# AY-Liu/Image-Editing-Framework

Hardware: AMD Instinct MI355X
Metric: denoising steps/sec (SD1.5 512x512 P2P edit step, UNet batch 4) (higher is better)
Workload: dtype f16x3; 1 GPU; sd15 UNet (859.5M params) P2P AttentionRefine edit step, 2 prompts x CFG = batch 4, 64x64 latents (512x512 px), 50-step DDIM, guidance 7.5, cross 0.8 / self 0.4, per-step null-text unconditional embeddings (P2P_NTI, edit_real.py); one independent edit per GPU; precision mode f16x3: fp32 storage; every contraction on split operands: hi + lo fp16 halves of each fp32 element, Ah Bh + Al Bh + Ah Bl =

## Files before the change

### image-editing-framework_amd/csrc/cross_p2p_x3.hip

```cpp
#include "ief_common.h"
#include "ief_params.h"
#include "x3_common.h"

template <int D, bool QS = false>
__global__ __launch_bounds__(256, (D > 80) ? 1 : 2) void attn_cross_p2p_x3_kernel(const IefAttnF32Params p, const int* __restrict__ edit_src,
                                                                                  const int* __restrict__ edit_slot,
                                                                                  const float* __restrict__ MT,
                                                                                  const float* __restrict__ coef) {
    constexpr int DG = (D + 15) / 16;
    constexpr int DT = (D + 31) / 32;
    constexpr int KLD = DG * 16 + 8;
    constexpr int VLD = 100;
    constexpr int MLD = 100;
    constexpr float SQ = 1.f, SK = 1.f, SV = 1.f, SP = 16384.f, SM = 256.f;
    const float SPE = p.p_scale > 0.f ? p.p_scale : SP;
    constexpr int RK = 2 * 96 * KLD, RV = 2 * DT * 32 * VLD, RM = 2 * 96 * MLD;
    constexpr int RSZ = RK > RV ? (RK > RM ? RK : RM) : (RV > RM ? RV : RM);
    __shared__ __attribute__((aligned(16))) half_t smem_c[RSZ];
    __shared__ float cf[2 * 96];
    half_t* Kh = smem_c;
    half_t* Kl = Kh + 96 * KLD;
    half_t* Vh = smem_c;
    half_t* Vl = Vh + DT * 32 * VLD;
    half_t* Mh = smem_c;
    half_t* Ml = Mh + 96 * MLD;
    const int tid = threadIdx.x, lane = tid & 63, wid = tid >> 6;
    const int li = lane & 31, lh = lane >> 5;
    const int nqb = gridDim.x;
    const int lid = xcd_remap(blockIdx.x + nqb * blockIdx.y, nqb * gridDim.y);
    const int bh = lid / nqb, qb = lid - bh * nqb, b = bh / p.heads, h = bh - b * p.heads;
    const int src = edit_src ? edit_src[b] : -1;
    const int qi = qb * 128 + wid * 32 + li;
    const int nt = (p.L + 31) / 32;
    const float sc2 = p.scale * 1.44269504088896341f / (SQ * SK);
    for (int c = tid; c < (int)(sizeof(smem_c) / 16); c += 256) ((f32x4*)smem_c)[c] = f32x4{0.f, 0.f, 0.f, 0.f};
    __syncthreads();

    constexpr int KCH = 32 * (D / 4);
    constexpr int NLD = (KCH + 255) / 256;
    auto probs = [&](int br, f32x16 (&P)[3]) {
        const float* Q = p.Q + (long long)(QS ? p.q_src[br] : br) * p.sQb + (long long)h * D;
        const float* Kp = p.K + (long long)br * p.sKb + (long long)h * D;
        half8_t qh[DG], ql[DG];
#pragma unroll
        for (int g = 0; g < DG; ++g) {
#pragma unroll
            for (int c2 = 0; c2 < 2; ++c2) {
                const int d0 = g * 16 + 8 * lh + 4 * c2;
                f32x4 v = {0.f, 0.f, 0.f, 0.f};
                if (qi < p.N && d0 < D) v = *(const f32x4*)(Q + (long long)qi * p.ldq + d0);
                half4 hh, ll;
                split4(v, SQ, hh, ll);
#pragma unroll
                for (int j = 0; j < 4; ++j) { qh[g][4 * c2 + j] = hh[j]; ql[g][4 * c2 + j] = ll[j]; }
            }
        }
        f32x4 rk[3][NLD];
#pragma unroll
        for (int t = 0; t < 3; ++t)
#pragma unroll
            for (int i = 0; i < NLD; ++i) {
                const int c = tid + 256 * i;
                const int row = c / (D / 4), ch = c - row * (D / 4);
                rk[t][i] = (t < nt && c < KCH && t * 32 + row < p.L) ? *(const f32x4*)(Kp + (long long)(t * 32 + row) * p.ldk + ch * 4)
                                                                     : f32x4{0.f, 0.f, 0.f, 0.f};
            }
        __syncthreads();
#pragma unroll
        for (int t = 0; t < 3; ++t)
#pragma unroll
            for (int i = 0; i < NLD; ++i) {
                const int c = tid + 256 * i;
                if (t < nt && c < KCH) {
                    const int row = c / (D / 4), ch = c - row * (D / 4);
                    half4 hh, ll;
                    split4(rk[t][i], SK, hh, ll);
                    *(half4*)(Kh + (t * 32 + row) * KLD + ch * 4) = hh;
                    *(half4*)(Kl + (t * 32 + row) * KLD + ch * 4) = ll;
                }
            }
        if (DG * 16 > D) {
            constexpr int PADC = (DG * 16 - D) / 4;
            for (int c = tid; c < 96 * PADC; c += 256) {
                const int row = c / PADC, ch = c - row * PADC;
                *(half4*)(Kh + row * KLD + D + ch * 4) = half4{0, 0, 0, 0};
                *(half4*)(Kl + row * KLD + D + ch * 4) = half4{0, 0, 0, 0};
            }
        }
        __syncthreads();
        float mx = -INFINITY;
#pragma unroll
        for (int t = 0; t < 3; ++t) {
#pragma unroll
            for (int r = 0; r < 16; ++r) P[t][r] = -INFINITY;
            if (t < nt) {
                f32x16 sacc;
#pragma unroll
                for (int r = 0; r < 16; ++r) sacc[r] = 0.f;
#pragma unroll
                for (int g = 0; g < DG; ++g) {
                    const half8_t kh = *(const half8_t*)(Kh + (t * 32 + li) * KLD + g * 16 + 8 * lh);
                    const half8_t kl = *(const half8_t*)(Kl + (t * 32 + li) * KLD + g * 16 + 8 * lh);
                    sacc = __builtin_amdgcn_mfma_f32_32x32x16_f16(kl, qh[g], sacc, 0, 0, 0);
                    sacc = __builtin_amdgcn_mfma_f32_32x32x16_f16(kh, ql[g], sacc, 0, 0, 0);
                    sacc = __builtin_amdgcn_mfma_f32_32x32x16_f16(kh, qh[g], sacc, 0, 0, 0);
                }
                if ((t + 1) * 32 > p.L) {
#pragma unroll
                    for (int r = 0; r < 16; ++r) {
                        const int key = t * 32 + (r & 3) + 8 * (r >> 2) + 4 * lh;
                        P[t][r] = key < p.L ? sacc[r] * sc2 : -INFINITY;
                        mx = fmaxf(mx, P[t][r]);
                    }
                } else {
#pragma unroll
                    for (int r = 0; r < 16; ++r) { P[t][r] = sacc[r] * sc2; mx = fmaxf(mx, P[t][r]); }
                }
            }
        }
        mx = fmaxf(mx, __shfl_xor(mx, 32));
        float ls = 0.f;
#pragma unroll
        for (int t = 0; t < 3; ++t)
#pragma unroll
            for (int r = 0; r < 16; ++r) { P[t][r] = __builtin_amdgcn_exp2f(P[t][r] - mx); ls += P[t][r]; }
        ls += __shfl_xor(ls, 32);
        const float inv = 1.0f / ls;
#pragma unroll
        for (int t = 0; t < 3; ++t)
#pragma unroll
            for (int r = 0; r < 16; ++r) P[t][r] *= inv;
    };
    auto split_p = [&](const f32x16& P, int s, half8_t& ph, half8_t& pl, float sp) {
#pragma unroll
        for (int c2 = 0; c2 < 2; ++c2) {
            const f32x4 v = {P[8 * s + 4 * c2], P[8 * s + 4 * c2 + 1], P[8 * s + 4 * c2 + 2], P[8 * s + 4 * c2 + 3]};
            half4 hh, ll;
            split4(v, sp, hh, ll);
#pragma unroll
            for (int j = 0; j < 4; ++j) { ph[4 * c2 + j] = hh[j]; pl[4 * c2 + j] = ll[j]; }
        }
    };

    f32x16 T[3];
    if (src >= 0) {
        const int slot = edit_slot[b];
        const float* mt = MT + (long long)slot * 96 * 96;
        f32x4 rm[9];
#pragma unroll
        for (int i = 0; i < 9; ++i) rm[i] = *(const f32x4*)(mt + (tid + 256 * i) * 4);
        if (tid < 192) cf[tid] = coef[(long long)slot * 192 + tid];
        f32x16 Ps[3];
        probs(src, Ps);
        __syncthreads();
#pragma unroll
        for (int i = 0; i < 9; ++i) {
            const int c = tid + 256 * i;
            const int w = c / 24, ch = c - w * 24;
            half4 hh, ll;
            split4(rm[i], SM, hh, ll);
            *(half4*)(Mh + w * MLD + ch * 4) = hh;
            *(half4*)(Ml + w * MLD + ch * 4) = ll;
        }
        __syncthreads();
        half8_t ph[6], pl[6];
#pragma unroll
        for (int s = 0; s < 6; ++s) split_p(Ps[s >> 1], s & 1, ph[s], pl[s], SP);
#pragma unroll
        for (int wt = 0; wt < 3; ++wt) {
#pragma unroll
            for (int r = 0; r < 16; ++r) T[wt][r] = 0.f;
#pragma unroll
            for (int s = 0; s < 6; ++s) {
                const half_t* mr = Mh + (wt * 32 + li) * MLD + 16 * s + 4 * lh;
                const half_t* mq = Ml + (wt * 32 + li) * MLD + 16 * s + 4 * lh;
                half8_t mh, ml;
                const half4 a0 = *(const half4*)mr, a1 = *(const half4*)(mr + 8);
                const half4 b0 = *(const half4*)mq, b1 = *(const half4*)(mq + 8);
#pragma unroll
                for (int j = 0; j < 4; ++j) { mh[j] = a0[j]; mh[4 + j] = a1[j]; ml[j] = b0[j]; ml[4 + j] = b1[j]; }
                T[wt] = __builtin_amdgcn_mfma_f32_32x32x16_f16(ml, ph[s], T[wt], 0, 0, 0);
                T[wt] = __builtin_amdgcn_mfma_f32_32x32x16_f16(mh, pl[s], T[wt], 0, 0, 0);
                T[wt] = __builtin_amdgcn_mfma_f32_32x32x16_f16(mh, ph[s], T[wt], 0, 0, 0);
            }
        }
    }
    const float* Vp = p.V + (long long)b * p.sVb + (long long)h * D;
    f32x4 rv[3][NLD];
#pragma unroll
    for (int t = 0; t < 3; ++t)
#pragma unroll
        for (int i = 0; i < NLD; ++i) {
            const int c = tid + 256 * i;
            const int row = c / (D / 4), ch = c - row * (D / 4);
            rv[t][i] = (t < nt && c < KCH && t * 32 + row < p.L) ? *(const f32x4*)(Vp + (long long)(t * 32 + row) * p.ldv + ch * 4)
                                                                 : f32x4{0.f, 0.f, 0.f, 0.f};
        }
    f32x16 P[3];
    probs(b, P);
    if (src >= 0) {
        const float invt = 1.0f / (SM * SP);
#pragma unroll
        for (int t = 0; t < 3; ++t)
#pragma unroll
            for (int r = 0; r < 16; ++r) {
                const int w = t * 32 + (r & 3) + 8 * (r >> 2) + 4 * lh;
                P[t][r] = cf[w] * (T[t][r] * invt) + cf[96 + w] * P[t][r];
            }
    }
    f32x16 o[DT];
#pragma unroll
    for (int tt = 0; tt < DT; ++tt)
#pragma unroll
        for (int r = 0; r < 16; ++r) o[tt][r] = 0.f;
    __syncthreads();
#pragma unroll
    for (int t = 0; t < 3; ++t)
#pragma unroll
        for (int i = 0; i < NLD; ++i) {
            const int c = tid + 256 * i;
            if (t < nt && c < KCH) {
                const int row = c / (D / 4), ch = c - row * (D / 4);
                half4 hh, ll;
                split4(rv[t][i], SV, hh, ll);
#pragma unroll
                for (int j = 0; j < 4; ++j) {
                    Vh[(ch * 4 + j) * VLD + t * 32 + row] = hh[j];
                    Vl[(ch * 4 + j) * VLD + t * 32 + row] = ll[j];
                }
            }
        }
    __syncthreads();
#pragma unroll
    for (int t = 0; t < 3; ++t) {
        if (t < nt) {
#pragma unroll
            for (int s = 0; s < 2; ++s) {
                half8_t ph, pl;
                split_p(P[t], s, ph, pl, SPE);
#pragma unroll
                for (int tt = 0; tt < DT; ++tt) {
                    const half_t* vr = Vh + (tt * 32 + li) * VLD + t * 32 + 16 * s + 4 * lh;
                    const half_t* vq = Vl + (tt * 32 + li) * VLD + t * 32 + 16 * s + 4 * lh;
                    half8_t vh, vl;
                    const half4 a0 = *(const half4*)vr, a1 = *(const half4*)(vr + 8);
                    const half4 b0 = *(const half4*)vq, b1 = *(const half4*)(vq + 8);
#pragma unroll
                    for (int j = 0; j < 4; ++j) { vh[j] = a0[j]; vh[4 + j] = a1[j]; vl[j] = b0[j]; vl[4 + j] = b1[j]; }
                    o[tt] = __builtin_amdgcn_mfma_f32_32x32x16_f16(vl, ph, o[tt], 0, 0, 0);
                    o[tt] = __builtin_amdgcn_mfma_f32_32x32x16_f16(vh, pl, o[tt], 0, 0, 0);
                    o[tt] = __builtin_amdgcn_mfma_f32_32x32x16_f16(vh, ph, o[tt], 0, 0, 0);
                }
            }
        }
    }
    const float inv = 1.0f / (SV * SPE);
    float* O = p.Out ? p.Out + (long long)b * p.sOb + (long long)h * D : nullptr;
    half_t* OP = p.OutP ? p.OutP + (long long)b * p.sOPb + (long long)h * D : nullptr;
    if (qi < p.N) {
#pragma unroll
        for (int tt = 0; tt < DT; ++tt)
#pragma unroll
            for (int g = 0; g < 4; ++g) {
                const int d = tt * 32 + 8 * g + 4 * lh;
                if (d < D) {
                    const f32x4 v = {o[tt][4 * g] * inv, o[tt][4 * g + 1] * inv, o[tt][4 * g + 2] * inv, o[tt][4 * g + 3] * inv};
                    if (O) *(f32x4*)(O + (long long)qi * p.ldo + d) = v;
                    if (OP) {
                        half4 hh, ll;
                        split4(v, 1.0f, hh, ll);
                        half_t* op = OP + (long long)qi * p.ldp + d;
                        *(half4*)op = hh;
                        *(half4*)(op + p.planeO) = ll;
                    }
                }
            }
    }
}

extern "C" int ief_attn_cross_p2p_f32(const IefAttnF32Params* pp, const int* edit_src, const int* edit_slot, const float* MT,
                                      const float* coef, void* stream) {
    if (!pp) return IEF_EINVAL;
    const IefAttnF32Params& p = *pp;
    if (!p.Q || !p.K || !p.V || (!p.Out && !p.OutP) || p.k_src || p.v_src) return IEF_EINVAL;
    if (p.OutP && ((p.ldp & 3) || (p.sOPb & 3) || (p.planeO & 3) || ((uintptr_t)p.OutP & 7))) return IEF_EALIGN;
    if (p.p_scale != 0.f && !(p.p_scale >= 1.f && p.p_scale <= 16384.f)) return IEF_EINVAL;
    if (edit_src && (!edit_slot || !MT || !coef)) return IEF_EINVAL;
    if (p.B <= 0 || p.heads <= 0 || p.N <= 0 || p.L <= 0 || p.L > 96) return IEF_ESHAPE;
    if ((p.ldq & 3) || (p.ldk & 3) || (p.ldv & 3) || (p.ldo & 3) || (p.sQb & 3) || (p.sKb & 3) || (p.sVb & 3) || (p.sOb & 3) ||
        (((uintptr_t)p.Q | (uintptr_t)p.K | (uintptr_t)p.V | (uintptr_t)(p.Out ? p.Out : p.Q) | (uintptr_t)(MT ? MT : p.Q)) & 15)) return IEF_EALIGN;
    if ((uintptr_t)p.q_src & 3) return IEF_EALIGN;
    hipStream_t st = (hipStream_t)stream;
    dim3 grid((p.N + 127) / 128, p.B * p.heads);
#define IEF_CROSS_X3_LAUNCH(D)                                                                                                  \
    if (p.q_src) hipLaunchKernelGGL((attn_cross_p2p_x3_kernel<D, true>), grid, dim3(256), 0, st, p, edit_src, edit_slot, MT, coef); \
    else hipLaunchKernelGGL((attn_cross_p2p_x3_kernel<D, false>), grid, dim3(256), 0, st, p, edit_src, edit_slot, MT, coef);       \
    break
    switch (p.d) {
        case 40: IEF_CROSS_X3_LAUNCH(40);
        case 64: IEF_CROSS_X3_LAUNCH(64);
        case 80: IEF_CROSS_X3_LAUNCH(80);
        case 160: IEF_CROSS_X3_LAUNCH(160);
        default: return IEF_ESHAPE;
    }
#undef IEF_CROSS_X3_LAUNCH
    IEF_LAUNCH_CHECK();
    return IEF_OK;
}
```

Before: 76.04 steps/s.

## Make cross-attention P2P x3 kernel persistent over query blocks with resident K/V/M

For head dims up to 80, the kernel now keeps the split K, source K, transposed V and mapping table resident in shared memory. It loops over several query blocks per workgroup, and the grid is sized from an assumed 256-CU count, so staging and splitting costs are amortised. It also prefetches the next block's Q while computing the current one, and uses 512-thread blocks for D<=64. This raises LDS use and register pressure, lowers occupancy, and adds an environment-variable override for the query-group count.

```diff
diff --git a/image-editing-framework_amd/csrc/cross_p2p_x3.hip b/image-editing-framework_amd/csrc/cross_p2p_x3.hip
--- a/image-editing-framework_amd/csrc/cross_p2p_x3.hip
+++ b/image-editing-framework_amd/csrc/cross_p2p_x3.hip
@@ -1,12 +1,21 @@
+#include <stdlib.h>
 #include "ief_common.h"
 #include "ief_params.h"
 #include "x3_common.h"
 
+template <int D>
+struct CrossX3 {
+    static constexpr bool RES = D <= 80;
+    static constexpr int NW = D <= 64 ? 8 : 4;
+    static constexpr int QB = 32 * NW;
+};
+
 template <int D, bool QS = false>
-__global__ __launch_bounds__(256, (D > 80) ? 1 : 2) void attn_cross_p2p_x3_kernel(const IefAttnF32Params p, const int* __restrict__ edit_src,
-                                                                                  const int* __restrict__ edit_slot,
-                                                                                  const float* __restrict__ MT,
-                                                                                  const float* __restrict__ coef) {
+__global__ __launch_bounds__(64 * CrossX3<D>::NW, CrossX3<D>::NW / 4) void attn_cross_p2p_x3_kernel(
+    const IefAttnF32Params p, const int* __restrict__ edit_src, const int* __restrict__ edit_slot, const float* __restrict__ MT,
+    const float* __restrict__ coef) {
+    constexpr bool RES = CrossX3<D>::RES;
+    constexpr int NT = 64 * CrossX3<D>::NW, QB = CrossX3<D>::QB;
     constexpr int DG = (D + 15) / 16;
     constexpr int DT = (D + 31) / 32;
     constexpr int KLD = DG * 16 + 8;
@@ -15,79 +24,135 @@
     constexpr float SQ = 1.f, SK = 1.f, SV = 1.f, SP = 16384.f, SM = 256.f;
     const float SPE = p.p_scale > 0.f ? p.p_scale : SP;
     constexpr int RK = 2 * 96 * KLD, RV = 2 * DT * 32 * VLD, RM = 2 * 96 * MLD;
-    constexpr int RSZ = RK > RV ? (RK > RM ? RK : RM) : (RV > RM ? RV : RM);
+    constexpr int OFK = RES ? RK : 0, OFV = RES ? 2 * RK : RK, OFM = RES ? 2 * RK + RV : RK;
+    constexpr int RSZ = RES ? 2 * RK + RV + RM : RK + (RV > RM ? RV : RM);
     __shared__ __attribute__((aligned(16))) half_t smem_c[RSZ];
     __shared__ float cf[2 * 96];
-    half_t* Kh = smem_c;
-    half_t* Kl = Kh + 96 * KLD;
-    half_t* Vh = smem_c;
-    half_t* Vl = Vh + DT * 32 * VLD;
-    half_t* Mh = smem_c;
-    half_t* Ml = Mh + 96 * MLD;
+    half_t* const Ksh = smem_c;
+    half_t* const Ksl = Ksh + 96 * KLD;
+    half_t* const Kh = smem_c + OFK;
+    half_t* const Kl = Kh + 96 * KLD;
+    half_t* const Vh = smem_c + OFV;
+    half_t* const Vl = Vh + DT * 32 * VLD;
+    half_t* const Mh = smem_c + OFM;
+    half_t* const Ml = Mh + 96 * MLD;
     const int tid = threadIdx.x, lane = tid & 63, wid = tid >> 6;
-    const int li = lane & 31, lh = lane >> 5;
-    const int nqb = gridDim.x;
-    const int lid = xcd_remap(blockIdx.x + nqb * blockIdx.y, nqb * gridDim.y);
-    const int bh = lid / nqb, qb = lid - bh * nqb, b = bh / p.heads, h = bh - b * p.heads;
+    int li = lane & 31, lh = lane >> 5, Lk = p.L;
+    const int G = gridDim.x;
+    const int nqb = (p.N + QB - 1) / QB;
+    const int lid = xcd_remap(blockIdx.x + G * blockIdx.y, G * gridDim.y);
+    const int bh = lid / G, g0 = lid - bh * G, b = bh / p.heads, h = bh - b * p.heads;
     const int src = edit_src ? edit_src[b] : -1;
-    const int qi = qb * 128 + wid * 32 + li;
+    const int slot = edit_src ? edit_slot[b] : 0;
     const int nt = (p.L + 31) / 32;
     const float sc2 = p.scale * 1.44269504088896341f / (SQ * SK);
-    for (int c = tid; c < (int)(sizeof(smem_c) / 16); c += 256) ((f32x4*)smem_c)[c] = f32x4{0.f, 0.f, 0.f, 0.f};
-    __syncthreads();
+    const float* const Qp = p.Q + (long long)(QS ? p.q_src[b] : b) * p.sQb + (long long)h * D;
 
     constexpr int KCH = 32 * (D / 4);
-    constexpr int NLD = (KCH + 255) / 256;
-    auto probs = [&](int br, f32x16 (&P)[3]) {
-        const float* Q = p.Q + (long long)(QS ? p.q_src[br] : br) * p.sQb + (long long)h * D;
-        const float* Kp = p.K + (long long)br * p.sKb + (long long)h * D;
-        half8_t qh[DG], ql[DG];
-#pragma unroll
-        for (int g = 0; g < DG; ++g) {
-#pragma unroll
-            for (int c2 = 0; c2 < 2; ++c2) {
-                const int d0 = g * 16 + 8 * lh + 4 * c2;
-                f32x4 v = {0.f, 0.f, 0.f, 0.f};
-                if (qi < p.N && d0 < D) v = *(const f32x4*)(Q + (long long)qi * p.ldq + d0);
-                half4 hh, ll;
-                split4(v, SQ, hh, ll);
-#pragma unroll
-                for (int j = 0; j < 4; ++j) { qh[g][4 * c2 + j] = hh[j]; ql[g][4 * c2 + j] = ll[j]; }
-            }
-        }
-        f32x4 rk[3][NLD];
+    constexpr int NLD = (KCH + NT - 1) / NT;
+    constexpr int MCH = 96 * 24;
+    constexpr int NM = (MCH + NT - 1) / NT;
+    auto load_kv = [&](const float* base, int ld, f32x4 (&r)[3][NLD]) {
 #pragma unroll
         for (int t = 0; t < 3; ++t)
 #pragma unroll
             for (int i = 0; i < NLD; ++i) {
-                const int c = tid + 256 * i;
+                const int c = tid + NT * i;
                 const int row = c / (D / 4), ch = c - row * (D / 4);
-                rk[t][i] = (t < nt && c < KCH && t * 32 + row < p.L) ? *(const f32x4*)(Kp + (long long)(t * 32 + row) * p.ldk + ch * 4)
-                                                                     : f32x4{0.f, 0.f, 0.f, 0.f};
-            }
-        __syncthreads();
+                r[t][i] = (t < nt && c < KCH && t * 32 + row < p.L) ? *(const f32x4*)(base + (long long)(t * 32 + row) * ld + ch * 4)
+                                                                    : f32x4{0.f, 0.f, 0.f, 0.f};
+            }
+    };
+    auto stage_k = [&](half_t* kh_, half_t* kl_, const f32x4 (&r)[3][NLD]) {
 #pragma unroll
         for (int t = 0; t < 3; ++t)
 #pragma unroll
             for (int i = 0; i < NLD; ++i) {
-                const int c = tid + 256 * i;
+                const int c = tid + NT * i;
                 if (t < nt && c < KCH) {
                     const int row = c / (D / 4), ch = c - row * (D / 4);
                     half4 hh, ll;
-                    split4(rk[t][i], SK, hh, ll);
-                    *(half4*)(Kh + (t * 32 + row) * KLD + ch * 4) = hh;
-                    *(half4*)(Kl + (t * 32 + row) * KLD + ch * 4) = ll;
+                    split4(r[t][i], SK, hh, ll);
+                    *(half4*)(kh_ + (t * 32 + row) * KLD + ch * 4) = hh;
+                    *(half4*)(kl_ + (t * 32 + row) * KLD + ch * 4) = ll;
                 }
             }
         if (DG * 16 > D) {
             constexpr int PADC = (DG * 16 - D) / 4;
-            for (int c = tid; c < 96 * PADC; c += 256) {
+            for (int c = tid; c < 96 * PADC; c += NT) {
                 const int row = c / PADC, ch = c - row * PADC;
-                *(half4*)(Kh + row * KLD + D + ch * 4) = half4{0, 0, 0, 0};
-                *(half4*)(Kl + row * KLD + D + ch * 4) = half4{0, 0, 0, 0};
-            }
-        }
-        __syncthreads();
+                *(half4*)(kh_ + row * KLD + D + ch * 4) = half4{0, 0, 0, 0};
+                *(half4*)(kl_ + row * KLD + D + ch * 4) = half4{0, 0, 0, 0};
+            }
+        }
+    };
+    auto stage_vt = [&](const f32x4 (&r)[3][NLD]) {
+#pragma unroll
+        for (int t = 0; t < 3; ++t)
+#pragma unroll
+            for (int i = 0; i < NLD; ++i) {
+                const int c = tid + NT * i;
+                if (t < nt && c < KCH) {
+                    const int row = c / (D / 4), ch = c - row * (D / 4);
+                    half4 hh, ll;
+                    split4(r[t][i], SV, hh, ll);
+#pragma unroll
+                    for (int j = 0; j < 4; ++j) {
+                        Vh[(ch * 4 + j) * VLD + t * 32 + row] = hh[j];
+                        Vl[(ch * 4 + j) * VLD + t * 32 + row] = ll[j];
+                    }
+                }
+            }
+        if (DT * 32 > D) {
+            constexpr int VCH = VLD / 4;
+            for (int c = tid; c < (DT * 32 - D) * VCH; c += NT) {
+                const int row = c / VCH, ch = c - row * VCH;
+                *(half4*)(Vh + (D + row) * VLD + ch * 4) = half4{0, 0, 0, 0};
+                *(half4*)(Vl + (D + row) * VLD + ch * 4) = half4{0, 0, 0, 0};
+            }
+        }
+    };
+    auto load_m = [&](const float* mt, f32x4 (&r)[NM]) {
+#pragma unroll
+        for (int i = 0; i < NM; ++i) {
+            const int c = tid + NT * i;
+            r[i] = c < MCH ? *(const f32x4*)(mt + c * 4) : f32x4{0.f, 0.f, 0.f, 0.f};
+        }
+    };
+    auto stage_m = [&](const f32x4 (&r)[NM]) {
+#pragma unroll
+        for (int i = 0; i < NM; ++i) {
+            const int c = tid + NT * i;
+            if (c < MCH) {
+                const int w = c / 24, ch = c - w * 24;
+                half4 hh, ll;
+                split4(r[i], SM, hh, ll);
+                *(half4*)(Mh + w * MLD + ch * 4) = hh;
+                *(half4*)(Ml + w * MLD + ch * 4) = ll;
+            }
+        }
+    };
+    auto load_q = [&](const float* Q, int qi, f32x4 (&r)[DG][2]) {
+#pragma unroll
+        for (int g = 0; g < DG; ++g)
+#pragma unroll
+            for (int c2 = 0; c2 < 2; ++c2) {
+                const int d0 = g * 16 + 8 * lh + 4 * c2;
+                r[g][c2] = (qi < p.N && d0 < D) ? *(const f32x4*)(Q + (long long)qi * p.ldq + d0) : f32x4{0.f, 0.f, 0.f, 0.f};
+            }
+    };
+    auto split_q = [&](const f32x4 (&r)[DG][2], half8_t (&qh)[DG], half8_t (&ql)[DG]) {
+#pragma unroll
+        for (int g = 0; g < DG; ++g)
+#pragma unroll
+            for (int c2 = 0; c2 < 2; ++c2) {
+                half4 hh, ll;
+                split4(r[g][c2], SQ, hh, ll);
+#pragma unroll
+                for (int j = 0; j < 4; ++j) { qh[g][4 * c2 + j] = hh[j]; ql[g][4 * c2 + j] = ll[j]; }
+            }
+    };
+    auto probs = [&](const half_t* kh_, const half_t* kl_, const half8_t (&qh)[DG], const half8_t (&ql)[DG], f32x16 (&P)[3]) {
         float mx = -INFINITY;
 #pragma unroll
         for (int t = 0; t < 3; ++t) {
@@ -99,17 +164,17 @@
                 for (int r = 0; r < 16; ++r) sacc[r] = 0.f;
 #pragma unroll
                 for (int g = 0; g < DG; ++g) {
-                    const half8_t kh = *(const half8_t*)(Kh + (t * 32 + li) * KLD + g * 16 + 8 * lh);
-                    const half8_t kl = *(const half8_t*)(Kl + (t * 32 + li) * KLD + g * 16 + 8 * lh);
+                    const half8_t kh = *(const half8_t*)(kh_ + (t * 32 + li) * KLD + g * 16 + 8 * lh);
+                    const half8_t kl = *(const half8_t*)(kl_ + (t * 32 + li) * KLD + g * 16 + 8 * lh);
                     sacc = __builtin_amdgcn_mfma_f32_32x32x16_f16(kl, qh[g], sacc, 0, 0, 0);
                     sacc = __builtin_amdgcn_mfma_f32_32x32x16_f16(kh, ql[g], sacc, 0, 0, 0);
                     sacc = __builtin_amdgcn_mfma_f32_32x32x16_f16(kh, qh[g], sacc, 0, 0, 0);
                 }
-                if ((t + 1) * 32 > p.L) {
+                if ((t + 1) * 32 > Lk) {
 #pragma unroll
                     for (int r = 0; r < 16; ++r) {
                         const int key = t * 32 + (r & 3) + 8 * (r >> 2) + 4 * lh;
-                        P[t][r] = key < p.L ? sacc[r] * sc2 : -INFINITY;
+                        P[t][r] = key < Lk ? sacc[r] * sc2 : -INFINITY;
                         mx = fmaxf(mx, P[t][r]);
                     }
                 } else {
@@ -141,28 +206,7 @@
             for (int j = 0; j < 4; ++j) { ph[4 * c2 + j] = hh[j]; pl[4 * c2 + j] = ll[j]; }
         }
     };
-
-    f32x16 T[3];
-    if (src >= 0) {
-        const int slot = edit_slot[b];
-        const float* mt = MT + (long long)slot * 96 * 96;
-        f32x4 rm[9];
-#pragma unroll
-        for (int i = 0; i < 9; ++i) rm[i] = *(const f32x4*)(mt + (tid + 256 * i) * 4);
-        if (tid < 192) cf[tid] = coef[(long long)slot * 192 + tid];
-        f32x16 Ps[3];
-        probs(src, Ps);
-        __syncthreads();
-#pragma unroll
-        for (int i = 0; i < 9; ++i) {
-            const int c = tid + 256 * i;
-            const int w = c / 24, ch = c - w * 24;
-            half4 hh, ll;
-            split4(rm[i], SM, hh, ll);
-            *(half4*)(Mh + w * MLD + ch * 4) = hh;
-            *(half4*)(Ml + w * MLD + ch * 4) = ll;
-        }
-        __syncthreads();
+    auto through_table = [&](const f32x16 (&Ps)[3], f32x16 (&T)[3]) {
         half8_t ph[6], pl[6];
 #pragma unroll
         for (int s = 0; s < 6; ++s) split_p(Ps[s >> 1], s & 1, ph[s], pl[s], SP);
@@ -184,98 +228,173 @@
                 T[wt] = __builtin_amdgcn_mfma_f32_32x32x16_f16(mh, ph[s], T[wt], 0, 0, 0);
             }
         }
+    };
+    float* const O = p.Out ? p.Out + (long long)b * p.sOb + (long long)h * D : nullptr;
+    half_t* const OP = p.OutP ? p.OutP + (long long)b * p.sOPb + (long long)h * D : nullptr;
+    auto mix_apply_store = [&](f32x16 (&P)[3], const f32x16 (&T)[3], int qi) {
+        if (src >= 0) {
+            const float invt = 1.0f / (SM * SP);
+#pragma unroll
+            for (int t = 0; t < 3; ++t)
+#pragma unroll
+                for (int r = 0; r < 16; ++r) {
+                    const int w = t * 32 + (r & 3) + 8 * (r >> 2) + 4 * lh;
+                    P[t][r] = cf[w] * (T[t][r] * invt) + cf[96 + w] * P[t][r];
+                }
+        }
+        f32x16 o[DT];
+#pragma unroll
+        for (int tt = 0; tt < DT; ++tt)
+#pragma unroll
+            for (int r = 0; r < 16; ++r) o[tt][r] = 0.f;
+#pragma unroll
+        for (int t = 0; t < 3; ++t) {
+            if (t < nt) {
+#pragma unroll
+                for (int s = 0; s < 2; ++s) {
+                    half8_t ph, pl;
+                    split_p(P[t], s, ph, pl, SPE);
+#pragma unroll
+                    for (int tt = 0; tt < DT; ++tt) {
+                        const half_t* vr = Vh + (tt * 32 + li) * VLD + t * 32 + 16 * s + 4 * lh;
+                        const half_t* vq = Vl + (tt * 32 + li) * VLD + t * 32 + 16 * s + 4 * lh;
+                        half8_t vh, vl;
+                        const half4 a0 = *(const half4*)vr, a1 = *(const half4*)(vr + 8);
+                        const half4 b0 = *(const half4*)vq, b1 = *(const half4*)(vq + 8);
+#pragma unroll
+                        for (int j = 0; j < 4; ++j) { vh[j] = a0[j]; vh[4 + j] = a1[j]; vl[j] = b0[j]; vl[4 + j] = b1[j]; }
+                        o[tt] = __builtin_amdgcn_mfma_f32_32x32x16_f16(vl, ph, o[tt], 0, 0, 0);
+                        o[tt] = __builtin_amdgcn_mfma_f32_32x32x16_f16(vh, pl, o[tt], 0, 0, 0);
+                        o[tt] = __builtin_amdgcn_mfma_f32_32x32x16_f16(vh, ph, o[tt], 0, 0, 0);
+                    }
+                }
+            }
+        }
+        const float inv = 1.0f / (SV * SPE);
+        if (qi < p.N) {
+#pragma unroll
+            for (int tt = 0; tt < DT; ++tt)
+#pragma unroll
+                for (int g = 0; g < 4; ++g) {
+                    const int d = tt * 32 + 8 * g + 4 * lh;
+                    if (d < D) {
+                        const f32x4 v = {o[tt][4 * g] * inv, o[tt][4 * g + 1] * inv, o[tt][4 * g + 2] * inv, o[tt][4 * g + 3] * inv};
+                        if (O) *(f32x4*)(O + (long long)qi * p.ldo + d) = v;
+                        if (OP) {
+                            half4 hh, ll;
+                            split4(v, 1.0f, hh, ll);
+                            half_t* op = OP + (long long)qi * p.ldp + d;
+                            *(half4*)op = hh;
+                            *(half4*)(op + p.planeO) = ll;
+                        }
+                    }
+                }
+        }
+    };
+
+    const float* const Kp = p.K + (long long)b * p.sKb + (long long)h * D;
+    const float* const Vp = p.V + (long long)b * p.sVb + (long long)h * D;
+    auto src_q = [&]() { return p.Q + (long long)(QS ? p.q_src[src] : src) * p.sQb + (long long)h * D; };
+    auto src_k = [&]() { return p.K + (long long)src * p.sKb + (long long)h * D; };
+    const float* Qsp = Qp;
+    int qb = g0, qi = qb * QB + wid * 32 + li;
+    f32x4 rq[DG][2];
+    half8_t qh[DG], ql[DG];
+    f32x16 T[3], P[3];
+    if constexpr (RES) {
+        f32x4 rqs[DG][2];
+        constexpr bool QFIRST = D <= 64;
+        {
+            f32x4 rks[3][NLD], rk[3][NLD], rv[3][NLD], rm[NM];
+            load_kv(Kp, p.ldk, rk);
+            load_kv(Vp, p.ldv, rv);
+            if (QFIRST) load_q(Qp, qi, rq);
+            if (src >= 0) {
+                Qsp = src_q();
+                load_kv(src_k(), p.ldk, rks);
+                load_m(MT + (long long)slot * 96 * 96, rm);
+                if (tid < 192) cf[tid] = coef[(long long)slot * 192 + tid];
+                if (QFIRST) load_q(Qsp, qi, rqs);
+            }
+            stage_k(Kh, Kl, rk);
+            stage_vt(rv);
+            if (src >= 0) {
+                stage_k(Ksh, Ksl, rks);
+                stage_m(rm);
+            }
+        }
+        if (!QFIRST) {
+            if (src >= 0) load_q(Qsp, qi, rqs);
+            load_q(Qp, qi, rq);
+        }
+        __syncthreads();
+        constexpr bool EARLY = D <= 64;
+        for (;;) {
+            asm volatile("" : "+v"(li), "+v"(lh), "+s"(Lk) : : "memory");
+            const int qbn = qb + G, qin = qbn * QB + wid * 32 + li;
+            if (src >= 0) {
+                split_q(rqs, qh, ql);
+                if (EARLY) load_q(Qsp, qin, rqs);
+                f32x16 Ps[3];
+                probs(Ksh, Ksl, qh, ql, Ps);
+                through_table(Ps, T);
+            }
+            split_q(rq, qh, ql);
+            if (EARLY) load_q(Qp, qin, rq);
+            probs(Kh, Kl, qh, ql, P);
+            if (!EARLY) load_q(Qp, qin, rq);
+            mix_apply_store(P, T, qi);
+            if (!EARLY && src >= 0) load_q(Qsp, qin, rqs);
+            if (qbn >= nqb) break;
+            qb = qbn;
+            qi = qin;
+        }
+    } else {
+        f32x4 rk[3][NLD], rv[3][NLD];
+        if (src >= 0) {
+            {
+                f32x4 rks[3][NLD], rm[NM];
+                load_kv(src_k(), p.ldk, rks);
+                load_m(MT + (long long)slot * 96 * 96, rm);
+                if (tid < 192) cf[tid] = coef[(long long)slot * 192 + tid];
+                load_q(src_q(), qi, rq);
+                stage_k(Ksh, Ksl, rks);
+                stage_m(rm);
+            }
+            __syncthreads();
+            load_kv(Kp, p.ldk, rk);
+            split_q(rq, qh, ql);
+            f32x16 Ps[3];
+            probs(Ksh, Ksl, qh, ql, Ps);
+            load_kv(Vp, p.ldv, rv);
+            through_table(Ps, T);
+            __syncthreads();
+        } else {
+            load_kv(Kp, p.ldk, rk);
+            load_kv(Vp, p.ldv, rv);
+        }
+        stage_k(Kh, Kl, rk);
+        load_q(Qp, qi, rq);
+        stage_vt(rv);
+        __syncthreads();
+        split_q(rq, qh, ql);
+        probs(Kh, Kl, qh, ql, P);
+        mix_apply_store(P, T, qi);
     }
-    const float* Vp = p.V + (long long)b * p.sVb + (long long)h * D;
-    f32x4 rv[3][NLD];
-#pragma unroll
-    for (int t = 0; t < 3; ++t)
-#pragma unroll
-        for (int i = 0; i < NLD; ++i) {
-            const int c = tid + 256 * i;
-            const int row = c / (D / 4), ch = c - row * (D / 4);
-            rv[t][i] = (t < nt && c < KCH && t * 32 + row < p.L) ? *(const f32x4*)(Vp + (long long)(t * 32 + row) * p.ldv + ch * 4)
-                                                                 : f32x4{0.f, 0.f, 0.f, 0.f};
-        }
-    f32x16 P[3];
-    probs(b, P);
-    if (src >= 0) {
-        const float invt = 1.0f / (SM * SP);
-#pragma unroll
-        for (int t = 0; t < 3; ++t)
-#pragma unroll
-            for (int r = 0; r < 16; ++r) {
-                const int w = t * 32 + (r & 3) + 8 * (r >> 2) + 4 * lh;
-                P[t][r] = cf[w] * (T[t][r] * invt) + cf[96 + w] * P[t][r];
-            }
-    }
-    f32x16 o[DT];
-#pragma unroll
-    for (int tt = 0; tt < DT; ++tt)
-#pragma unroll
-        for (int r = 0; r < 16; ++r) o[tt][r] = 0.f;
-    __syncthreads();
-#pragma unroll
-    for (int t = 0; t < 3; ++t)
-#pragma unroll
-        for (int i = 0; i < NLD; ++i) {
-            const int c = tid + 256 * i;
-            if (t < nt && c < KCH) {
-                const int row = c / (D / 4), ch = c - row * (D / 4);
-                half4 hh, ll;
-                split4(rv[t][i], SV, hh, ll);
-#pragma unroll
-                for (int j = 0; j < 4; ++j) {
-                    Vh[(ch * 4 + j) * VLD + t * 32 + row] = hh[j];
-                    Vl[(ch * 4 + j) * VLD + t * 32 + row] = ll[j];
-                }
-            }
-        }
-    __syncthreads();
-#pragma unroll
-    for (int t = 0; t < 3; ++t) {
-        if (t < nt) {
-#pragma unroll
-            for (int s = 0; s < 2; ++s) {
-                half8_t ph, pl;
-                split_p(P[t], s, ph, pl, SPE);
-#pragma unroll
-                for (int tt = 0; tt < DT; ++tt) {
-                    const half_t* vr = Vh + (tt * 32 + li) * VLD + t * 32 + 16 * s + 4 * lh;
-                    const half_t* vq = Vl + (tt * 32 + li) * VLD + t * 32 + 16 * s + 4 * lh;
-                    half8_t vh, vl;
-                    const half4 a0 = *(const half4*)vr, a1 = *(const half4*)(vr + 8);
-                    const half4 b0 = *(const half4*)vq, b1 = *(const half4*)(vq + 8);
-#pragma unroll
-                    for (int j = 0; j < 4; ++j) { vh[j] = a0[j]; vh[4 + j] = a1[j]; vl[j] = b0[j]; vl[4 + j] = b1[j]; }
-                    o[tt] = __builtin_amdgcn_mfma_f32_32x32x16_f16(vl, ph, o[tt], 0, 0, 0);
-                    o[tt] = __builtin_amdgcn_mfma_f32_32x32x16_f16(vh, pl, o[tt], 0, 0, 0);
-                    o[tt] = __builtin_amdgcn_mfma_f32_32x32x16_f16(vh, ph, o[tt], 0, 0, 0);
-                }
-            }
-        }
-    }
-    const float inv = 1.0f / (SV * SPE);
-    float* O = p.Out ? p.Out + (long long)b * p.sOb + (long long)h * D : nullptr;
-    half_t* OP = p.OutP ? p.OutP + (long long)b * p.sOPb + (long long)h * D : nullptr;
-    if (qi < p.N) {
-#pragma unroll
-        for (int tt = 0; tt < DT; ++tt)
-#pragma unroll
-            for (int g = 0; g < 4; ++g) {
-                const int d = tt * 32 + 8 * g + 4 * lh;
-                if (d < D) {
-                    const f32x4 v = {o[tt][4 * g] * inv, o[tt][4 * g + 1] * inv, o[tt][4 * g + 2] * inv, o[tt][4 * g + 3] * inv};
-                    if (O) *(f32x4*)(O + (long long)qi * p.ldo + d) = v;
-                    if (OP) {
-                        half4 hh, ll;
-                        split4(v, 1.0f, hh, ll);
-                        half_t* op = OP + (long long)qi * p.ldp + d;
-                        *(half4*)op = hh;
-                        *(half4*)(op + p.planeO) = ll;
-                    }
-                }
-            }
-    }
+}
+
+#define IEF_CROSS_X3_CUS 256
+
+static int cross_x3_qgroups(int nqb, long long groups, bool resident) {
+    if (!resident) return nqb;
+    const char* e = getenv("IEF_CROSS_X3_QGROUPS");
+    const int forced = e ? atoi(e) : 0;
+    if (forced > 0) return forced < nqb ? forced : nqb;
+    long long g = IEF_CROSS_X3_CUS / groups;
+    if (g < 1) g = 1;
+    if (g > nqb) g = nqb;
+    const int iters = (nqb + (int)g - 1) / (int)g;
+    return (nqb + iters - 1) / iters;
 }
 
 extern "C" int ief_attn_cross_p2p_f32(const IefAttnF32Params* pp, const int* edit_src, const int* edit_slot, const float* MT,
@@ -291,10 +410,14 @@
         (((uintptr_t)p.Q | (uintptr_t)p.K | (uintptr_t)p.V | (uintptr_t)(p.Out ? p.Out : p.Q) | (uintptr_t)(MT ? MT : p.Q)) & 15)) return IEF_EALIGN;
     if ((uintptr_t)p.q_src & 3) return IEF_EALIGN;
     hipStream_t st = (hipStream_t)stream;
-    dim3 grid((p.N + 127) / 128, p.B * p.heads);
-#define IEF_CROSS_X3_LAUNCH(D)                                                                                                  \
-    if (p.q_src) hipLaunchKernelGGL((attn_cross_p2p_x3_kernel<D, true>), grid, dim3(256), 0, st, p, edit_src, edit_slot, MT, coef); \
-    else hipLaunchKernelGGL((attn_cross_p2p_x3_kernel<D, false>), grid, dim3(256), 0, st, p, edit_src, edit_slot, MT, coef);       \
+    const long long groups = (long long)p.B * p.heads;
+#define IEF_CROSS_X3_LAUNCH(D)                                                                                                   \
+    {                                                                                                                            \
+        const int nqb = (p.N + CrossX3<D>::QB - 1) / CrossX3<D>::QB;                                                             \
+        const dim3 grid(cross_x3_qgroups(nqb, groups, CrossX3<D>::RES), (unsigned)groups), block(64 * CrossX3<D>::NW);           \
+        if (p.q_src) hipLaunchKernelGGL((attn_cross_p2p_x3_kernel<D, true>), grid, block, 0, st, p, edit_src, edit_slot, MT, coef); \
+        else hipLaunchKernelGGL((attn_cross_p2p_x3_kernel<D, false>), grid, block, 0, st, p, edit_src, edit_slot, MT, coef);       \
+    }                                                                                                                            \
     break
     switch (p.d) {
         case 40: IEF_CROSS_X3_LAUNCH(40);
```

Measured after the change: 76.53 steps/s (median of 6 runs). About the same (+0.6%).
